# cordum-io/cordum

Measured on AMD Instinct MI355X. Metric: jobs dispatched/sec (whole node), higher is better.
Workload: dtype int64-bitset/int32 (control-plane integer path); 1 GPU; model=cordum control-plane dispatch pipeline (echo workers), global_batch=16384, seq_len=256, parallelism=shard1, rules=1024, workers_per_rank=1000, denied_jobs=14465

## Files before the change

cordum_amd/ops/hip/cordum_kernels.hip:

```cpp
#include <hip/hip_runtime.h>
#include <cstdint>

#define WAVE 64
#define BLOCK 256


template <int W, int JPT>
__global__ __launch_bounds__(BLOCK) void policy_first_match_kernel(
    const long long* __restrict__ rule_any,
    const long long* __restrict__ rule_all,
    const signed char* __restrict__ rule_secrets,
    const long long* __restrict__ rule_mcp,
    const unsigned char* __restrict__ rule_mcp_any,
    const long long* __restrict__ job_any,
    const long long* __restrict__ job_all,
    const unsigned char* __restrict__ job_secrets,
    const long long* __restrict__ job_mcp,
    const unsigned char* __restrict__ job_mcp_used,
    int* __restrict__ out_first,
    int R, int J, int rules_per_chunk)
{
    const int rule_chunk_begin = blockIdx.y * rules_per_chunk;
    const int rule_chunk_end = min(R, rule_chunk_begin + rules_per_chunk);
    constexpr int ANY_W = 7 * W;
// ... 986 lines not shown
    }
}

__global__ __launch_bounds__(BLOCK) void policy_first_match_mfma_kernel(
    const signed char* __restrict__ a_pack,
    const signed char* __restrict__ b_pack,
    const int* __restrict__ cards,
    const signed char* __restrict__ rule_secrets,
    const unsigned char* __restrict__ job_secrets,
    const int* __restrict__ tile_dims,
    int* __restrict__ out_first,
    int J, int R, int tiles_per_chunk)
{
    const int lane = threadIdx.x % WAVE;
    const int jt = blockIdx.x;
    v4i afrag[1][9];
    #pragma unroll
    for (int d = 0; d < 9; ++d)
        afrag[0][d] = *(const v4i*)&a_pack[(((size_t)jt * 9 + d) * 64 + lane) * 16];
    mfma_first_match_tiles<1>(afrag, b_pack, cards, rule_secrets, job_secrets,
                              tile_dims, out_first, J, R, tiles_per_chunk);
}

template <int TJ>
__global__ __launch_bounds__(BLOCK) void policy_first_match_mfma_bits_kernel(
    const long long* __restrict__ any_bits,
    const long long* __restrict__ all_bits,
    const signed char* __restrict__ b_pack,
    const int* __restrict__ cards,
    const signed char* __restrict__ rule_secrets,
    const unsigned char* __restrict__ job_secrets,
    const int* __restrict__ tile_dims,
    int* __restrict__ out_first,
    int J, int R, int tiles_per_chunk)
{
    const int lane = threadIdx.x % WAVE;
    const int shift = (lane >> 4) * 16;
    v4i afrag[TJ][9];
    #pragma unroll
    for (int t = 0; t < TJ; ++t) {
        const int job = (blockIdx.x * TJ + t) * 16 + (lane & 15);
        #pragma unroll
        for (int d = 0; d < 9; ++d) {
            unsigned long long w = 0;
            if (job < J)
                w = (unsigned long long)(d < 7 ? any_bits[(size_t)job * 7 + d]
                                               : all_bits[(size_t)job * 2 + (d - 7)]);
            const unsigned int slice = (unsigned int)(w >> shift) & 0xFFFFu;
            #pragma unroll
            for (int q = 0; q < 4; ++q)
                afrag[t][d][q] = (int)((((slice >> (4 * q)) & 0xFu) * 0x00204081u) & 0x01010101u);
        }
    }
    mfma_first_match_tiles<TJ>(afrag, b_pack, cards, rule_secrets, job_secrets,
                               tile_dims, out_first, J, R, tiles_per_chunk);
}


__global__ __launch_bounds__(BLOCK) void policy_gate_kernel(
    const int* __restrict__ first,
    const signed char* __restrict__ decisions,
    signed char* __restrict__ out_decision,
    int* __restrict__ denied_slots,
    int* __restrict__ denied_count,
    int* __restrict__ allowed_slots,
    int* __restrict__ allowed_count,
    int J, int R)
{
// ... 889 lines not shown
}

void tick_prologue(torch::Tensor states, torch::Tensor counts,
                   c10::optional<torch::Tensor> first,
                   torch::Tensor w_active, torch::Tensor w_maxp,
                   torch::Tensor w_cpu, torch::Tensor w_gpu, torch::Tensor out_keys)
{
    CHECK_DEV(states);
    const int B = (int)states.size(0);
    const int n = (int)counts.size(0);
    const int NW = (int)out_keys.size(0);
    TORCH_CHECK(w_active.size(0) == NW && w_maxp.size(0) == NW &&
                w_cpu.size(0) == NW && w_gpu.size(0) == NW, "worker table size mismatch");
    TORCH_CHECK(!first.has_value() || first->size(0) == B, "first must be [B]");
    const int blocks = (std::max(std::max(B, n), std::max(NW, 1)) + BLOCK - 1) / BLOCK;
    hipLaunchKernelGGL(tick_prologue_kernel, dim3(blocks), dim3(BLOCK), 0, cur_stream(),
        states.data_ptr<uint8_t>(), B, counts.data_ptr<int>(), n,
        first.has_value() ? first->data_ptr<int>() : (int*)nullptr,
        w_active.data_ptr<int>(), w_maxp.data_ptr<int>(),
        w_cpu.data_ptr<float>(), w_gpu.data_ptr<float>(),
        (unsigned long long*)out_keys.data_ptr<int64_t>(), NW);
}

void policy_first_match_mfma_bits_into(
    torch::Tensor any_bits, torch::Tensor all_bits,
    torch::Tensor b_pack, torch::Tensor cards,
    torch::Tensor rule_secrets, torch::Tensor job_secrets,
    torch::Tensor tile_dims, int64_t n_rules, torch::Tensor out, int64_t job_tiles)
{
    CHECK_DEV(any_bits); CHECK_DEV(b_pack);
    CHECK_CONTIG(any_bits); CHECK_CONTIG(all_bits);
    TORCH_CHECK(job_tiles == 1 || job_tiles == 2, "job_tiles must be 1 or 2");
    TORCH_CHECK(any_bits.dim() == 3 && any_bits.size(1) == 7 && any_bits.size(2) == 1 &&
                all_bits.dim() == 3 && all_bits.size(1) == 2 && all_bits.size(2) == 1,
                "MFMA K1 needs the 1-word vocab: any [J,7,1], all [J,2,1]");
    const int J = (int)any_bits.size(0), R = (int)n_rules;
    TORCH_CHECK(all_bits.size(0) == J && job_secrets.size(0) >= J && out.size(0) >= J,
                "job tensors must cover J");
    const int TJ = (int)job_tiles;
    const int Jt = ((J + 15) / 16 + TJ - 1) / TJ;
    const int Rt = (R + 15) / 16;
    if (J == 0 || R == 0) return;
    TORCH_CHECK(b_pack.size(0) >= Rt && tile_dims.size(0) >= Rt &&
                rule_secrets.size(0) >= Rt * 16 && cards.size(0) >= Rt * 16,
                "rule pack smaller than n_rules");
    int nchunks = std::max(1, std::min((Rt + 3) / 4, std::max(1, 2048 / std::max(Jt, 1))));
    const int tiles_per_chunk = (Rt + nchunks - 1) / nchunks;
    auto launch = [&](auto kernel) {
        hipLaunchKernelGGL(kernel, dim3(Jt, nchunks), dim3(BLOCK), 0, cur_stream(),
            (const long long*)any_bits.data_ptr<int64_t>(),
            (const long long*)all_bits.data_ptr<int64_t>(),
            (const signed char*)b_pack.data_ptr<int8_t>(),
            cards.data_ptr<int>(),
            (const signed char*)rule_secrets.data_ptr<int8_t>(),
            job_secrets.data_ptr<uint8_t>(),
            tile_dims.data_ptr<int>(),
            out.data_ptr<int>(), J, R, tiles_per_chunk);
    };
    if (TJ == 2) launch(policy_first_match_mfma_bits_kernel<2>);
    else launch(policy_first_match_mfma_bits_kernel<1>);
}

void gate_route(torch::Tensor first, torch::Tensor decisions, torch::Tensor out_decision,
                torch::Tensor denied_slots, torch::Tensor denied_count,
                torch::Tensor allowed_slots, torch::Tensor allowed_count,
                torch::Tensor states, torch::Tensor deadlines,
                torch::Tensor dlq_ring, torch::Tensor dlq_head,
                torch::Tensor pick, torch::Tensor order, torch::Tensor valid_count,
                torch::Tensor j_poolmask, torch::Tensor j_labels,
                int64_t full_mask, int64_t K,
                torch::Tensor routable_slots, torch::Tensor routable_widx,
                torch::Tensor routable_count, torch::Tensor extra_zero)
{
    CHECK_DEV(first);
    const int J = (int)first.size(0);
    TORCH_CHECK(out_decision.size(0) >= J && denied_slots.size(0) >= J &&
                allowed_slots.size(0) >= J && states.size(0) >= J &&
                deadlines.size(0) >= J && pick.size(0) >= J &&
                j_poolmask.size(0) >= J && j_labels.size(0) >= J &&
                routable_slots.size(0) >= J && routable_widx.size(0) >= J,
                "per-job tensors must cover J");
    TORCH_CHECK(K <= order.size(0), "K exceeds the order table");
    const int n_extra = (int)extra_zero.size(0);
// ... 388 lines not shown
            arow[dim_topic * W + w] = ol[o_idx * W + w];
            arow[dim_risk * W + w] = has_risk ? rl[r_idx * W + w] : 0;
            lrow[all_requires * W + w] = has_req ? ql[q_idx * W + w] : 0;
        }
    }
}

void synthetic_fresh_stamped(torch::Tensor any_bits,
                             torch::Tensor all_bits,
                             torch::Tensor tenant_lut, torch::Tensor topic_lut,
                             torch::Tensor risk_lut, torch::Tensor req_lut,
                             int64_t seed, int64_t step,
                             int64_t dim_tenant, int64_t dim_topic, int64_t dim_risk,
                             int64_t all_requires,
                             c10::optional<torch::Tensor> payload,
                             int64_t payload_words,
                             int64_t threads, int64_t isa_cap)
{
    TORCH_CHECK(!any_bits.is_cuda() && !all_bits.is_cuda(),
                "synthetic_fresh_stamped is a host encoder");
    CHECK_CONTIG(any_bits); CHECK_CONTIG(all_bits);
    CHECK_CONTIG(tenant_lut); CHECK_CONTIG(topic_lut);
    CHECK_CONTIG(risk_lut); CHECK_CONTIG(req_lut);
    cordum_enc::EncodeJob a;
    a.B = any_bits.size(0);
    a.W = any_bits.size(2);
    a.V = tenant_lut.size(0);
    TORCH_CHECK(any_bits.size(1) == 7 && all_bits.size(0) == a.B &&
                all_bits.size(1) == 2 && all_bits.size(2) == a.W, "bad batch shape");
    for (const torch::Tensor* l : {&tenant_lut, &topic_lut, &risk_lut, &req_lut})
        TORCH_CHECK(l->size(0) == a.V && l->size(1) == a.W, "bad LUT shape");
    TORCH_CHECK(dim_tenant >= 0 && dim_tenant < 7 && dim_topic >= 0 && dim_topic < 7 &&
                dim_risk >= 0 && dim_risk < 7 && all_requires >= 0 && all_requires < 2,
                "dim index out of range");
    a.any = any_bits.data_ptr<int64_t>();
    a.all = all_bits.data_ptr<int64_t>();
    a.tenant_lut = tenant_lut.data_ptr<int64_t>();
    a.topic_lut = topic_lut.data_ptr<int64_t>();
    a.risk_lut = risk_lut.data_ptr<int64_t>();
    a.req_lut = req_lut.data_ptr<int64_t>();
    a.seed = (uint64_t)seed;
    a.step = (uint64_t)step;
    a.dim_tenant = (int)dim_tenant;
    a.dim_topic = (int)dim_topic;
    a.dim_risk = (int)dim_risk;
    a.all_requires = (int)all_requires;
    a.payload = nullptr;
    a.payload_words = payload_words;
    if (payload.has_value()) {
        TORCH_CHECK(!payload->is_cuda() && payload->is_contiguous() &&
                    payload->scalar_type() == torch::kInt32 && payload_words > 0 &&
                    payload->numel() >= a.B * payload_words, "bad payload ring buffer");
        a.payload = payload->data_ptr<int32_t>();
    }
    cordum_enc::encode_batch(a, (int)threads, (int)isa_cap);
}

void pack_jobs_mfma_dev(torch::Tensor any_bits, torch::Tensor all_bits,
                        torch::Tensor a_pack)
{
    const int B = (int)any_bits.size(0);
    const int Jt = (int)a_pack.size(0);
    const int n = Jt * 9 * 64;
    const int blocks = (n + BLOCK - 1) / BLOCK;
    hipLaunchKernelGGL(pack_jobs_mfma_kernel, dim3(blocks), dim3(BLOCK), 0, cur_stream(),
        (const long long*)any_bits.data_ptr<int64_t>(),
        (const long long*)all_bits.data_ptr<int64_t>(),
        a_pack.data_ptr<int8_t>(), B, Jt);
}

// ... 27 lines not shown
    m.def("load_feedback", &load_feedback, "per-worker active-count histogram");
    m.def("run_readiness", &run_readiness, "K3 run/step readiness sweep");
    m.def("synthetic_fresh", &synthetic_fresh,
          py::call_guard<py::gil_scoped_release>(),
          "fused host synthetic-batch encoder");
    m.def("pack_jobs_mfma_dev", &pack_jobs_mfma_dev, "device job packing for the MFMA K1");
    m.def("synthetic_fresh_stamped", &synthetic_fresh_stamped,
          py::call_guard<py::gil_scoped_release>(),
          "host batch preparation in one call: synthetic dims + payload step stamp",
          py::arg("any_bits"), py::arg("all_bits"), py::arg("tenant_lut"),
          py::arg("topic_lut"), py::arg("risk_lut"), py::arg("req_lut"),
          py::arg("seed"), py::arg("step"), py::arg("dim_tenant"), py::arg("dim_topic"),
          py::arg("dim_risk"), py::arg("all_requires"), py::arg("payload"),
          py::arg("payload_words"), py::arg("threads") = 1, py::arg("isa_cap") = -1);
    m.def("encoder_isa_level", [] { return cordum_enc::max_isa_level(); },
          "widest encoder ISA this CPU runs (0 baseline, 1 AVX2, 2 AVX-512DQ)");
    m.def("tick_prologue", &tick_prologue,
          "fused tick 1/5: PENDING re-admit + counter reset + first prime + worker keys");
    m.def("policy_first_match_mfma_bits_into", &policy_first_match_mfma_bits_into,
          "fused tick 3/5: K1 MFMA with A fragments built from the staged bit words",
          py::arg("any_bits"), py::arg("all_bits"), py::arg("b_pack"), py::arg("cards"),
          py::arg("rule_secrets"), py::arg("job_secrets"), py::arg("tile_dims"),
          py::arg("n_rules"), py::arg("out"), py::arg("job_tiles") = 1);
    m.def("gate_route", &gate_route,
          "fused tick 4/5: gate + DENIED/DLQ + spread/exact pick + routable compaction");
    m.def("tick_finish", &tick_finish,
          "fused tick 5/5: echo + state chain + load feedback + counter fold");
    m.def("pack_by_dest", &pack_by_dest, "padded per-destination dispatch pack");
    m.def("pack_requeue", &pack_requeue, "redeliver last tick's requeue ring into the send segments");
    m.def("wf_sweep", &wf_sweep, "K3-WF readiness sweep + approval holds + condition/delay commits");
    m.def("wf_expand", &wf_expand, "K3-WF for_each/worker child expansion into the child arena");
    m.def("wf_apply", &wf_apply, "K3-WF child result application with failure injection");
    m.def("wf_apply_dead", &wf_apply_dead, "K3-WF dead-letter child application");
    m.def("wf_commit", &wf_commit, "K3-WF step aggregation + retry/backoff commit");
    m.def("wf_timeout_scan", &wf_timeout_scan, "K4-WF stale-step timeout scan");
    m.def("wf_readmit", &wf_readmit, "K3-WF continuous run re-admission from template");
    m.def("wf_status", &wf_status, "K3-WF run status roll-up");
    m.def("wf_grant", &wf_grant, "K3-WF host approval grants");
    m.def("materialize_rq_payload", &materialize_rq_payload, "copy requeued payload rows into the rq arena");
    m.def("gather_payload_padded", &gather_payload_padded, "payload gather into padded send arena");
    m.def("echo_padded", &echo_padded, "region-valid echo over padded recv arena");
    m.def("apply_transitions_padded", &apply_transitions_padded, "K5 over padded slot list");
    m.def("load_feedback_padded", &load_feedback_padded, "padded per-worker load histogram");
    m.def("set_transition_lut", &set_transition_lut, "upload transition legality LUT");
    m.def("apply_transitions", &apply_transitions, "K5 batched state transitions");
    m.def("deadline_scan", &deadline_scan, "K4 deadline/staleness scan");
// ... 3 lines not shown
```

cordum_amd/ops/hip/synthetic_encode.h:

```cpp
#pragma once

#include <cstddef>
#include <cstdint>
#include <thread>

namespace cordum_enc {

struct EncodeJob {
    int64_t* any;
    int64_t* all;
    const int64_t* tenant_lut;
    const int64_t* topic_lut;
    const int64_t* risk_lut;
    const int64_t* req_lut;
    int64_t B, W, V;
    uint64_t seed, step;
    int dim_tenant, dim_topic, dim_risk, all_requires;
    int32_t* payload;
    int64_t payload_words;
};

constexpr int kBlock = 64;
constexpr uint32_t kRiskCut = 1288490189u;
constexpr uint32_t kReqCut = 429496730u;

static inline uint64_t splitmix64(uint64_t x) {
    x += 0x9E3779B97F4A7C15ull;
    x = (x ^ (x >> 30)) * 0xBF58476D1CE4E5B9ull;
    x = (x ^ (x >> 27)) * 0x94D049BB133111EBull;
    return x ^ (x >> 31);
}

static inline uint64_t batch_base(uint64_t seed, uint64_t step) {
    return splitmix64(seed * 0x5851F42D4C957F2Dull ^ step);
}

__attribute__((always_inline)) static inline void encode_range_impl(
    const EncodeJob& a, int64_t i0, int64_t i1)
{
    const uint64_t base = batch_base(a.seed, a.step);
    const uint64_t v = (uint64_t)a.V;
    const int64_t W = a.W;
    const int32_t stamp = (int32_t)(uint32_t)a.step;
    uint32_t t_idx[kBlock], o_idx[kBlock], r_idx[kBlock], q_idx[kBlock];
    uint32_t c_risk[kBlock], c_req[kBlock];
    for (int64_t b0 = i0; b0 < i1; b0 += kBlock) {
        const int n = (int)((i1 - b0) < kBlock ? (i1 - b0) : kBlock);
        for (int k = 0; k < kBlock; ++k) {
            const uint64_t h0 = splitmix64(base ^ (uint64_t)(b0 + k));
            const uint64_t h1 = splitmix64(h0);
            const uint64_t h2 = splitmix64(h1);
            t_idx[k] = (uint32_t)(((h0 & 0xffffffffull) * v) >> 32);
            o_idx[k] = (uint32_t)(((h0 >> 32) * v) >> 32);
            r_idx[k] = (uint32_t)(((h1 & 0xffffffffull) * v) >> 32);
            q_idx[k] = (uint32_t)(((h1 >> 32) * v) >> 32);
            c_risk[k] = (uint32_t)h2;
            c_req[k] = (uint32_t)(h2 >> 32);
        }
        if (W == 1) {
            int64_t* arow = a.any + (size_t)b0 * 7;
            int64_t* lrow = a.all + (size_t)b0 * 2;
            for (int k = 0; k < n; ++k, arow += 7, lrow += 2) {
                arow[a.dim_tenant] = a.tenant_lut[t_idx[k]];
                arow[a.dim_topic] = a.topic_lut[o_idx[k]];
                arow[a.dim_risk] = c_risk[k] < kRiskCut ? a.risk_lut[r_idx[k]] : 0;
                lrow[a.all_requires] = c_req[k] < kReqCut ? a.req_lut[q_idx[k]] : 0;
            }
        } else {
            for (int k = 0; k < n; ++k) {
                int64_t* arow = a.any + (size_t)(b0 + k) * 7 * W;
                int64_t* lrow = a.all + (size_t)(b0 + k) * 2 * W;
                const bool has_risk = c_risk[k] < kRiskCut;
                const bool has_req = c_req[k] < kReqCut;
                const int64_t* tl = a.tenant_lut + (size_t)t_idx[k] * W;
                const int64_t* ol = a.topic_lut + (size_t)o_idx[k] * W;
                const int64_t* rl = a.risk_lut + (size_t)r_idx[k] * W;
                const int64_t* ql = a.req_lut + (size_t)q_idx[k] * W;
                for (int64_t w = 0; w < W; ++w) {
                    arow[a.dim_tenant * W + w] = tl[w];
                    arow[a.dim_topic * W + w] = ol[w];
                    arow[a.dim_risk * W + w] = has_risk ? rl[w] : 0;
                    lrow[a.all_requires * W + w] = has_req ? ql[w] : 0;
// ... 62 lines not shown
```

cordum_amd/ops/pipeline.py:

```python
from __future__ import annotations

import time
from dataclasses import dataclass
from typing import List, Optional

import torch
import torch.distributed as dist

from ..protocol.states import transition_lut
from ..safety import policy as pol
from . import get_ext
from .policy_compile import CompiledPolicy, JobBatch, JobEncoder, compile_policy, first_match_reference

UNSPECIFIED, PENDING, APPROVAL, SCHEDULED, DISPATCHED, RUNNING = 0, 1, 2, 3, 4, 5
SUCCEEDED, FAILED, CANCELLED, TIMEOUT, DENIED = 6, 7, 8, 9, 10

ALLOW_CODES = (1, 5)


@dataclass
class TickStats:
    completed: int = 0
    denied: int = 0
    unrouted: int = 0
# ... 43 lines not shown

    def __init__(self, compiled: CompiledPolicy, vocab: int = 48, seed: int = 5):
        from .policy_compile import ALL_REQUIRES, DIM_RISK, DIM_TENANT, DIM_TOPIC

        enc = JobEncoder(compiled)
        W = compiled.words
        rows = []
        for v in range(vocab):
            jb = enc.encode([
                pol.PolicyInput(tenant=f"t{v}", topic=f"job.a{v}",
                                risk_tags=[f"tag{v}"], requires=[f"req{v}"])
            ])
            rows.append(jb)
        self.W = W
        self.vocab = vocab
        self.tenant_lut = torch.stack([r.any_bits[0, DIM_TENANT] for r in rows])
        self.topic_lut = torch.stack([r.any_bits[0, DIM_TOPIC] for r in rows])
        self.risk_lut = torch.stack([r.any_bits[0, DIM_RISK] for r in rows])
        self.req_lut = torch.stack([r.all_bits[0, ALL_REQUIRES] for r in rows])
        self.gen = torch.Generator().manual_seed(seed)
        self.seed = seed
        self._dims = (DIM_TENANT, DIM_TOPIC, DIM_RISK, ALL_REQUIRES)
        self._bufs = None

    def _scratch(self, J: int):
        if self._bufs is not None and self._bufs[0].shape[0] == J:
            return self._bufs
        W = self.W
        self._bufs = (
            torch.zeros(J, dtype=torch.int64),
            torch.zeros(J, dtype=torch.int64),
            torch.zeros(J, dtype=torch.int64),
            torch.zeros(J, dtype=torch.int64),
            torch.zeros(J, dtype=torch.float32),
            torch.zeros(J, dtype=torch.float32),
            torch.zeros((J, W), dtype=torch.int64),
            torch.zeros((J, 1), dtype=torch.int64),
        )
        return self._bufs

    def fresh(self, out: JobBatch) -> None:
        DIM_TENANT, DIM_TOPIC, DIM_RISK, ALL_REQUIRES = self._dims
        J = out.n_jobs
        g = self.gen
        t_idx, o_idx, r_idx, q_idx, u_risk, u_req, row, mask = self._scratch(J)
        t_idx.random_(0, self.vocab, generator=g)
# ... 24 lines not shown
        DIM_TENANT, DIM_TOPIC, DIM_RISK, ALL_REQUIRES = self._dims
        ext.synthetic_fresh(out.any_bits, out.all_bits,
                            self.tenant_lut, self.topic_lut,
                            self.risk_lut, self.req_lut,
                            self.seed, step,
                            DIM_TENANT, DIM_TOPIC, DIM_RISK, ALL_REQUIRES)

    encode_threads = 1

    def fresh_stamped(self, out: JobBatch, step: int, ext, payload: torch.Tensor,
                      payload_words: int, threads: Optional[int] = None,
                      isa_cap: int = -1) -> None:
        DIM_TENANT, DIM_TOPIC, DIM_RISK, ALL_REQUIRES = self._dims
        ext.synthetic_fresh_stamped(out.any_bits, out.all_bits,
                                    self.tenant_lut, self.topic_lut,
                                    self.risk_lut, self.req_lut,
                                    self.seed, step,
                                    DIM_TENANT, DIM_TOPIC, DIM_RISK, ALL_REQUIRES,
                                    payload, payload_words,
                                    self.encode_threads if threads is None else threads,
                                    isa_cap)


class _RefOps:

    def __init__(self):
        self._lut = None

    def set_transition_lut(self, lut):
        self._lut = lut

    def policy_first_match(self, rule_any, rule_all, rule_secrets, rule_mcp, rule_mcp_any,
                           job_any, job_all, job_secrets, job_mcp, job_mcp_used, chunks):
        from types import SimpleNamespace

        c = SimpleNamespace(any_masks=rule_any, all_masks=rule_all, secrets=rule_secrets,
                            mcp_masks=rule_mcp, mcp_any=rule_mcp_any,
                            n_rules=int(rule_any.shape[0]))
        b = SimpleNamespace(any_bits=job_any, all_bits=job_all, secrets=job_secrets,
                            mcp_bits=job_mcp, mcp_used=job_mcp_used,
                            n_jobs=int(job_any.shape[0]))
        return first_match_reference(c, b)

    def worker_precompute(self, w_pool, w_active, w_maxp, w_cpu, w_gpu):
        from .reference import worker_precompute_ref

# ... 254 lines not shown
    nbytes = ((n64 * 8 + 2 * B + 7) // 8) * 8
    if pin:
        buf = torch.zeros(nbytes, dtype=torch.uint8).pin_memory()
    else:
        buf = torch.zeros(nbytes, dtype=torch.uint8, device=device)
    o = 0

    def take64(*shape):
        nonlocal o
        n = 1
        for s in shape:
            n *= s
        t = buf[o:o + n * 8].view(torch.int64).view(*shape)
        o += n * 8
        return t

    any_b = take64(B, 7, W)
    all_b = take64(B, 2, W)
    mcp_b = take64(B, 4, W)
    sec = buf[o:o + B]
    o += B
    used = buf[o:o + B]
    return JobBatch(any_b, all_b, sec, mcp_b, used), buf


def alloc_result_block(B: int, device=None, pin: bool = False):
    nbytes = ((4 * B + 16 + B + 7) // 8) * 8
    if pin:
        buf = torch.zeros(nbytes, dtype=torch.uint8).pin_memory()
    else:
        buf = torch.zeros(nbytes, dtype=torch.uint8, device=device)
    sums = buf[0:4 * B].view(torch.int32)
    counts = buf[4 * B:4 * B + 16].view(torch.int32)
    dec = buf[4 * B + 16:5 * B + 16].view(torch.int8)
    return sums, counts, dec, buf


class DevicePipeline:
    def __init__(
        self,
        device: torch.device,
        batch_size: int = 16384,
        n_local_workers: int = 1000,
        n_rules: int = 1024,
        payload_words: int = 64,
        world_size: int = 1,
        rank: int = 0,
        n_batches: int = 8,
        policy: Optional[pol.SafetyPolicy] = None,
        seed: int = 7,
        backend: str = "ext",
        use_mfma: Optional[bool] = None,
        mfma_pack_on_device: bool = False,
        pad_cap: Optional[int] = None,
        unfused_tick: bool = False,
        k1_job_tiles: int = 2,
    ):
        self._k1_job_tiles = k1_job_tiles
        self._pad_cap_override = pad_cap
        self._unfused_tick = unfused_tick
        self._mfma_device_pack = mfma_pack_on_device
        device = torch.device(device)
        self.ext = _RefOps() if backend == "ref" else get_ext(required=True)
        self.device = device
        self.B = batch_size
        self.NWL = n_local_workers
        self.world = world_size
        self.rank = rank
        self.payload_words = payload_words

        self.ext.set_transition_lut(torch.tensor(transition_lut(), dtype=torch.uint8).flatten())

        policy = policy or make_synthetic_policy(n_rules, seed=seed)
        for w in (1, 2, 4):
            self.compiled = compile_policy(policy, words=w)
            if self.compiled.exact:
                break
        assert self.compiled.exact, "bench policy must compile exactly"
        self.cpol = self.compiled.to(device)

# ... 98 lines not shown
            ):
                a_pack, _ = pack_jobs_mfma(jb_host)
                self.mfma_a_packs.append(a_pack.to(device))
        self._fused_capable = device.type == "cuda" and self.world == 1 and backend != "ref"
        self._tick = 0
        self.total_completed = 0
        self.total_denied = 0


    def _spread(self, pick):
        full_mask = (1 << self.world) - 1
        K = min(int(self.order_buf.shape[0]), 1024)
        self.ext.spread_pick(self.order_buf, self.valid_buf, self.j_poolmask,
                             self.j_labels, full_mask, pick, K)
        return pick

    def _refresh_order(self) -> None:
        if self._tick % 8 != 1:
            return
        self.order_buf.copy_(torch.argsort(self.w_keys).to(torch.int32))
        valid = ((self.w_keys >> 32) & 0xFFFFFFFF).ne(0xFFFFFFFE)
        self.valid_buf.copy_(valid.sum().to(torch.int32).reshape(1))

    def _fused_body(self, slot: int) -> None:
        if self._unfused_tick:
            return self._unfused_body(slot)
        B = self.B
        ext = self.ext
        jb = self.batches[slot]
        full_mask = (1 << self.world) - 1
        ext.tick_prologue(self.states, self._counts,
                          self.first_buf if self._use_mfma else None,
                          self.w_active_local, self.w_maxp,
                          self.w_cpu_local, self.w_gpu_local, self.w_keys)
        ext.least_loaded_pick_into(self.w_pool, self.w_keys, self.w_labels,
                                   self.j_poolmask, self.j_labels,
                                   self.valid_buf, full_mask, self.pick_buf)
        if self._use_mfma:
            ext.policy_first_match_mfma_bits_into(
                jb.any_bits, jb.all_bits, self.mfma_policy.b_pack,
                self.mfma_policy.cards, self.mfma_policy.secrets, jb.secrets,
                self.mfma_policy.tile_dims, self.compiled.n_rules, self.first_buf,
                self._k1_job_tiles)
            first = self.first_buf
        else:
            first = ext.policy_first_match(
                self.cpol.any_masks, self.cpol.all_masks, self.cpol.secrets,
                self.cpol.mcp_masks, self.cpol.mcp_any,
                jb.any_bits, jb.all_bits, jb.secrets, jb.mcp_bits, jb.mcp_used, 0,
            )
        K = min(int(self.order_buf.shape[0]), 1024)
        ext.gate_route(first, self.cpol.decisions, self.out_decision,
                       self.denied_slots, self.denied_count,
                       self.allowed_slots, self.allowed_count,
                       self.states, self.deadlines, self.dlq_ring, self.dlq_head,
                       self.pick_buf, self.order_buf, self.valid_buf,
                       self.j_poolmask, self.j_labels, full_mask, K,
                       self.routable_slots, self.routable_widx,
                       self.routable_count, self.w_active_local)
        ext.tick_finish(self.payloads[slot], self.routable_slots,
                        self.routable_widx, self.routable_count,
                        self.res_arena[: B * self.payload_words], self.res_sums,
                        self.payload_words,
                        self.states, self.attempts, self.deadlines,
                        [SCHEDULED, DISPATCHED, RUNNING, SUCCEEDED],
                        self.w_active_local, self.NWL, self.rank,
                        self._counts, self.acc_counts, B)

    def _unfused_body(self, slot: int) -> None:
        B = self.B
        ext = self.ext
        jb = self.batches[slot]
        if self._use_mfma:
            ext.begin_tick_first(self.states, self._counts, self.first_buf)
            if self._mfma_device_pack:
                ext.pack_jobs_mfma_dev(jb.any_bits, jb.all_bits,
                                       self.mfma_a_packs[slot])
            ext.policy_first_match_mfma_into(
                self.mfma_a_packs[slot], self.mfma_policy.b_pack, self.mfma_policy.cards,
                self.mfma_policy.secrets, jb.secrets, self.mfma_policy.tile_dims,
                self.B, self.compiled.n_rules, self.first_buf,
            )
            first = self.first_buf
# ... 76 lines not shown
        )
        self.total_completed += stats.completed
        self.total_denied += stats.denied
        return stats

    def ensure_e2e(self, seed: int = 11, payload_ring: int = 4) -> None:
        if hasattr(self, "_e2e_enc"):
            return
        assert not self._use_mfma or self._mfma_device_pack, \
            "e2e ingest needs staged descriptors: bitset K1 or device-packed MFMA"
        self._e2e_enc = SyntheticEncoder(self.compiled, seed=seed + self.rank)
        pin = self.device.type == "cuda"
        B, W = self.B, self.compiled.words

        def host(shape, dtype):
            t = torch.zeros(shape, dtype=dtype)
            return t.pin_memory() if pin else t

        self._e2e_host = JobBatch(
            host((B, 7, W), torch.int64), host((B, 2, W), torch.int64),
            host((B,), torch.uint8), host((B, 4, W), torch.int64),
            host((B,), torch.uint8),
        )
        g = torch.Generator().manual_seed(seed * 31 + self.rank)
        self._e2e_payloads = []
        for _ in range(payload_ring):
            p = torch.randint(-(1 << 31), (1 << 31) - 1,
                              (B * self.payload_words,), dtype=torch.int32, generator=g)
            self._e2e_payloads.append(p.pin_memory() if pin else p)
        self._e2e_step = 0

    def _encode_host(self, s: int, hb: JobBatch, enc: SyntheticEncoder,
                     payload: torch.Tensor) -> None:
        if hasattr(self.ext, "synthetic_fresh_stamped"):
            enc.fresh_stamped(hb, s, self.ext, payload, self.payload_words)
            return
        if hasattr(self.ext, "synthetic_fresh"):
            enc.fresh_fast(hb, s, self.ext)
        else:
            enc.fresh(hb)
        payload.view(self.B, self.payload_words)[:, 0] = s

    def tick_e2e(self) -> TickStats:
        self.ensure_e2e()
        t0 = time.perf_counter()
        step = self._e2e_step
        self._e2e_step += 1
        payload = self._e2e_payloads[step % len(self._e2e_payloads)]
        self._encode_host(step, self._e2e_host, self._e2e_enc, payload)
        nb = self.device.type == "cuda"
        jb = self.batches[0]
        jb.any_bits.copy_(self._e2e_host.any_bits, non_blocking=nb)
# ... 63 lines not shown
            if cuda:
                torch.cuda.synchronize(self.device)
            lats[s] = time.perf_counter() - t_enc[s]
        return completed, denied, lats

    def e2e_run(self, steps: int):
        self.ensure_e2e()
        if self.world > 1:
            return self._e2e_run_dist(steps)
        if self.device.type != "cuda" or not self._fused_capable:
            completed = denied = 0
            lats = []
            for _ in range(steps):
                st = self.tick_e2e()
                completed += st.completed
                denied += st.denied
                lats.append(st.wall_s)
            return completed, denied, lats

        self._ensure_graphs()
        B = self.B
        nslots = 2
        nhost = 4
        if not hasattr(self, "_e2e_hosts2"):
            Wc = self.compiled.words
            pairs = [alloc_batch_staging(B, Wc, pin=True) for _ in range(nhost)]
            self._e2e_hosts2 = [p[0] for p in pairs]
            self._e2e_host_bufs = [p[1] for p in pairs]
            self._e2e_encs = [SyntheticEncoder(self.compiled, seed=101 + 13 * i + self.rank)
                              for i in range(nhost)]
            outs = [alloc_result_block(B, pin=True) for _ in range(nslots)]
            self._e2e_out_sums = [o[0] for o in outs]
            self._e2e_out_counts = [o[1] for o in outs]
            self._e2e_out_dec = [o[2] for o in outs]
            self._e2e_out_blocks = [o[3] for o in outs]
            self._e2e_ev = [torch.cuda.Event() for _ in range(nslots)]
            self._e2e_in_ev = [torch.cuda.Event() for _ in range(nslots)]
            self._e2e_copy_stream = torch.cuda.Stream(device=self.device)
            from concurrent.futures import ThreadPoolExecutor

            self._e2e_pool = ThreadPoolExecutor(max_workers=2)

        completed = denied = 0
        lats = [0.0] * steps
        t_enc = [0.0] * steps

        def encode(s: int):
            t_enc[s] = time.perf_counter()
            self._encode_host(s, self._e2e_hosts2[s % nhost], self._e2e_encs[s % nhost],
                              self._e2e_payloads[s % len(self._e2e_payloads)])

        def harvest(s_prev: int) -> None:
            nonlocal completed, denied
            slot = s_prev % nslots
            self._e2e_ev[slot].synchronize()
            c = self._e2e_out_counts[slot]
            denied_n = int(c[0])
            routable = int(c[2])
            completed += routable
            denied += denied_n
            lats[s_prev] = time.perf_counter() - t_enc[s_prev]
            self._e2e_sums = self._e2e_out_sums[slot]
            self._e2e_decisions = self._e2e_out_dec[slot]

        futs = {}

        def submit(s: int) -> None:
            if s < steps:
                futs[s] = self._e2e_pool.submit(encode, s)

        submit(0)
        submit(1)
        for s in range(steps):
            futs.pop(s).result()
            slot = s % nslots
            with torch.cuda.stream(self._e2e_copy_stream):
                self.batch_bufs[slot].copy_(
                    self._e2e_host_bufs[s % nhost], non_blocking=True)
                self.payloads[slot].copy_(
                    self._e2e_payloads[s % len(self._e2e_payloads)],
                    non_blocking=True)
                self._e2e_in_ev[slot].record(self._e2e_copy_stream)
            torch.cuda.current_stream(self.device).wait_event(self._e2e_in_ev[slot])
            self._graphs[slot].replay()
            self._e2e_out_blocks[slot].copy_(self._res_block, non_blocking=True)
            self._e2e_ev[slot].record()
            submit(s + 2)
            if s >= 1:
                harvest(s - 1)
        harvest(steps - 1)
        return completed, denied, lats

    def tick(self) -> TickStats:
        if getattr(self, "_fused_capable", False):
            return self._tick_fused()
        if self.world > 1:
            return self._tick_padded()
        return self._tick_eager()

    def reset_stats(self) -> None:
        self.acc_counts.zero_()
        self.total_completed = 0
        self.total_denied = 0

    def tick_async(self) -> None:
        if getattr(self, "_fused_capable", False):
            self._ensure_graphs()
# ... 370 lines not shown
```

cordum_amd/ops/policy_mfma.py:

```python
from __future__ import annotations

from dataclasses import dataclass
from typing import Tuple

import torch

from .policy_compile import CompiledPolicy, JobBatch

N_DIMS = 9
VOCAB = 64


def _bits_to_onehot(words: torch.Tensor) -> torch.Tensor:
    n, d, w = words.shape
    assert w == 1, "MFMA variant supports 1-word (vocab<=64) policies"
    shifts = torch.arange(64, dtype=torch.int64)
    return ((words >> shifts.view(1, 1, 64)) & 1).to(torch.int8)


def _pack_a(onehot: torch.Tensor) -> torch.Tensor:
    J = onehot.shape[0]
    Jt = (J + 15) // 16
    padded = torch.zeros(Jt * 16, N_DIMS, VOCAB, dtype=torch.int8)
    padded[:J] = onehot
    a = padded.view(Jt, 16, N_DIMS, 4, 16)
    a = a.permute(0, 2, 3, 1, 4).reshape(Jt, N_DIMS, 64, 16)
    return a.contiguous()


def _pack_b(onehot: torch.Tensor) -> torch.Tensor:
    R = onehot.shape[0]
    Rt = (R + 15) // 16
    padded = torch.zeros(Rt * 16, N_DIMS, VOCAB, dtype=torch.int8)
    padded[:R] = onehot
    b = padded.view(Rt, 16, N_DIMS, 4, 16)
    b = b.permute(0, 2, 3, 1, 4)
    b = b.reshape(Rt, N_DIMS, 64, 16)
    return b.contiguous()


@dataclass
class MfmaPolicy:
    b_pack: torch.Tensor
    cards: torch.Tensor
    secrets: torch.Tensor
    tile_dims: torch.Tensor
    n_rules: int

    def to(self, device):
        return MfmaPolicy(self.b_pack.to(device), self.cards.to(device),
                          self.secrets.to(device), self.tile_dims.to(device),
                          self.n_rules)


def pack_policy_mfma(c: CompiledPolicy) -> MfmaPolicy:
    assert c.words == 1, "MFMA variant needs vocab <= 64"
    R = c.n_rules
    rule_bits = torch.cat([c.any_masks, c.all_masks], dim=1)
    onehot = _bits_to_onehot(rule_bits)
    b_pack = _pack_b(onehot)
    Rt = b_pack.shape[0]
    cards = torch.zeros(Rt * 16, N_DIMS, dtype=torch.int32)
    cards[:R] = onehot.sum(dim=2).to(torch.int32)
    if Rt * 16 > R:
        cards[R:, 7] = 127
    secrets = torch.full((Rt * 16,), -1, dtype=torch.int8)
    secrets[:R] = c.secrets
    used = (cards.view(Rt, 16, N_DIMS) != 0).any(dim=1)
    tile_dims = (used.to(torch.int32) << torch.arange(N_DIMS, dtype=torch.int32)).sum(
        dim=1).to(torch.int32)
    return MfmaPolicy(b_pack, cards, secrets, tile_dims, R)


def pack_jobs_mfma(jobs: JobBatch) -> Tuple[torch.Tensor, torch.Tensor]:
    job_bits = torch.cat([jobs.any_bits, jobs.all_bits], dim=1)
    onehot = _bits_to_onehot(job_bits)
    return _pack_a(onehot), jobs.secrets


def first_match_mfma(ext, mp: MfmaPolicy, a_pack: torch.Tensor,
                     job_secrets: torch.Tensor, n_jobs: int) -> torch.Tensor:
    return ext.policy_first_match_mfma(
        a_pack, mp.b_pack, mp.cards, mp.secrets, job_secrets, mp.tile_dims,
        int(n_jobs), int(mp.n_rules),
    )
```

Baseline: 110.1 million jobs/s.

## Stage jobs in compact columnar wire layout with single H2D copy per step

Adds a wire layout that holds only the policy-live dimension columns, the payload and optional secrets in one contiguous pinned buffer. The host encoder writes straight into this columnar layout, and a new MFMA K1 variant reads those columns directly. The e2e loop then does one host-to-device copy per step instead of two, through separately captured graphs. The aim is to cut PCIe bytes and host encode work for dims no rule uses, at the cost of another code path and a second set of captured graphs.

```diff
diff --git a/cordum_amd/ops/hip/cordum_kernels.hip b/cordum_amd/ops/hip/cordum_kernels.hip
--- a/cordum_amd/ops/hip/cordum_kernels.hip
+++ b/cordum_amd/ops/hip/cordum_kernels.hip
@@ -1032,7 +1032,7 @@
                               tile_dims, out_first, J, R, tiles_per_chunk);
 }
 
-template <int TJ>
+template <int TJ, bool COLS>
 __global__ __launch_bounds__(BLOCK) void policy_first_match_mfma_bits_kernel(
     const long long* __restrict__ any_bits,
     const long long* __restrict__ all_bits,
@@ -1042,7 +1042,7 @@
     const unsigned char* __restrict__ job_secrets,
     const int* __restrict__ tile_dims,
     int* __restrict__ out_first,
-    int J, int R, int tiles_per_chunk)
+    int J, int R, int tiles_per_chunk, unsigned live)
 {
     const int lane = threadIdx.x % WAVE;
     const int shift = (lane >> 4) * 16;
@@ -1053,7 +1053,11 @@
         #pragma unroll
         for (int d = 0; d < 9; ++d) {
             unsigned long long w = 0;
-            if (job < J)
+            if (COLS) {
+                if (job < J && ((live >> d) & 1u))
+                    w = (unsigned long long)any_bits[
+                        (size_t)__builtin_popcount(live & ((1u << d) - 1u)) * J + job];
+            } else if (job < J)
                 w = (unsigned long long)(d < 7 ? any_bits[(size_t)job * 7 + d]
                                                : all_bits[(size_t)job * 2 + (d - 7)]);
             const unsigned int slice = (unsigned int)(w >> shift) & 0xFFFFu;
@@ -1989,21 +1993,16 @@
         (unsigned long long*)out_keys.data_ptr<int64_t>(), NW);
 }
 
-void policy_first_match_mfma_bits_into(
-    torch::Tensor any_bits, torch::Tensor all_bits,
+static void launch_mfma_bits(
+    const long long* words, const long long* all_words, bool cols, unsigned live, int J,
     torch::Tensor b_pack, torch::Tensor cards,
     torch::Tensor rule_secrets, torch::Tensor job_secrets,
     torch::Tensor tile_dims, int64_t n_rules, torch::Tensor out, int64_t job_tiles)
 {
-    CHECK_DEV(any_bits); CHECK_DEV(b_pack);
-    CHECK_CONTIG(any_bits); CHECK_CONTIG(all_bits);
+    CHECK_DEV(b_pack);
     TORCH_CHECK(job_tiles == 1 || job_tiles == 2, "job_tiles must be 1 or 2");
-    TORCH_CHECK(any_bits.dim() == 3 && any_bits.size(1) == 7 && any_bits.size(2) == 1 &&
-                all_bits.dim() == 3 && all_bits.size(1) == 2 && all_bits.size(2) == 1,
-                "MFMA K1 needs the 1-word vocab: any [J,7,1], all [J,2,1]");
-    const int J = (int)any_bits.size(0), R = (int)n_rules;
-    TORCH_CHECK(all_bits.size(0) == J && job_secrets.size(0) >= J && out.size(0) >= J,
-                "job tensors must cover J");
+    const int R = (int)n_rules;
+    TORCH_CHECK(job_secrets.size(0) >= J && out.size(0) >= J, "job tensors must cover J");
     const int TJ = (int)job_tiles;
     const int Jt = ((J + 15) / 16 + TJ - 1) / TJ;
     const int Rt = (R + 15) / 16;
@@ -2015,17 +2014,59 @@
     const int tiles_per_chunk = (Rt + nchunks - 1) / nchunks;
     auto launch = [&](auto kernel) {
         hipLaunchKernelGGL(kernel, dim3(Jt, nchunks), dim3(BLOCK), 0, cur_stream(),
-            (const long long*)any_bits.data_ptr<int64_t>(),
-            (const long long*)all_bits.data_ptr<int64_t>(),
+            words, all_words,
             (const signed char*)b_pack.data_ptr<int8_t>(),
             cards.data_ptr<int>(),
             (const signed char*)rule_secrets.data_ptr<int8_t>(),
             job_secrets.data_ptr<uint8_t>(),
             tile_dims.data_ptr<int>(),
-            out.data_ptr<int>(), J, R, tiles_per_chunk);
+            out.data_ptr<int>(), J, R, tiles_per_chunk, live);
     };
-    if (TJ == 2) launch(policy_first_match_mfma_bits_kernel<2>);
-    else launch(policy_first_match_mfma_bits_kernel<1>);
+    if (cols) {
+        if (TJ == 2) launch(policy_first_match_mfma_bits_kernel<2, true>);
+        else launch(policy_first_match_mfma_bits_kernel<1, true>);
+    } else {
+        if (TJ == 2) launch(policy_first_match_mfma_bits_kernel<2, false>);
+        else launch(policy_first_match_mfma_bits_kernel<1, false>);
+    }
+}
+
+void policy_first_match_mfma_bits_into(
+    torch::Tensor any_bits, torch::Tensor all_bits,
+    torch::Tensor b_pack, torch::Tensor cards,
+    torch::Tensor rule_secrets, torch::Tensor job_secrets,
+    torch::Tensor tile_dims, int64_t n_rules, torch::Tensor out, int64_t job_tiles)
+{
+    CHECK_DEV(any_bits);
+    CHECK_CONTIG(any_bits); CHECK_CONTIG(all_bits);
+    TORCH_CHECK(any_bits.dim() == 3 && any_bits.size(1) == 7 && any_bits.size(2) == 1 &&
+                all_bits.dim() == 3 && all_bits.size(1) == 2 && all_bits.size(2) == 1,
+                "MFMA K1 needs the 1-word vocab: any [J,7,1], all [J,2,1]");
+    const int J = (int)any_bits.size(0);
+    TORCH_CHECK(all_bits.size(0) == J, "job tensors must cover J");
+    launch_mfma_bits((const long long*)any_bits.data_ptr<int64_t>(),
+                     (const long long*)all_bits.data_ptr<int64_t>(), false, 0u, J,
+                     b_pack, cards, rule_secrets, job_secrets, tile_dims, n_rules, out,
+                     job_tiles);
+}
+
+void policy_first_match_mfma_cols_into(
+    torch::Tensor cols, int64_t live,
+    torch::Tensor b_pack, torch::Tensor cards,
+    torch::Tensor rule_secrets, torch::Tensor job_secrets,
+    torch::Tensor tile_dims, int64_t n_rules, torch::Tensor out, int64_t job_tiles)
+{
+    CHECK_DEV(cols); CHECK_CONTIG(cols);
+    TORCH_CHECK(cols.scalar_type() == torch::kInt64 && cols.dim() == 2,
+                "cols must be int64 [n_live, J]");
+    TORCH_CHECK(live >= 0 && live < (1 << 9), "live is a 9-bit dim mask");
+    TORCH_CHECK(cols.size(0) == __builtin_popcount((unsigned)live),
+                "cols needs one row per live dim");
+    CHECK_DEV(job_secrets);
+    launch_mfma_bits((const long long*)cols.data_ptr<int64_t>(), nullptr, true,
+                     (unsigned)live, (int)cols.size(1),
+                     b_pack, cards, rule_secrets, job_secrets, tile_dims, n_rules, out,
+                     job_tiles);
 }
 
 void gate_route(torch::Tensor first, torch::Tensor decisions, torch::Tensor out_decision,
@@ -2460,7 +2501,7 @@
     CHECK_CONTIG(any_bits); CHECK_CONTIG(all_bits);
     CHECK_CONTIG(tenant_lut); CHECK_CONTIG(topic_lut);
     CHECK_CONTIG(risk_lut); CHECK_CONTIG(req_lut);
-    cordum_enc::EncodeJob a;
+    cordum_enc::EncodeJob a{};
     a.B = any_bits.size(0);
     a.W = any_bits.size(2);
     a.V = tenant_lut.size(0);
@@ -2484,6 +2525,62 @@
     a.dim_risk = (int)dim_risk;
     a.all_requires = (int)all_requires;
     a.payload = nullptr;
+    a.payload_words = payload_words;
+    if (payload.has_value()) {
+        TORCH_CHECK(!payload->is_cuda() && payload->is_contiguous() &&
+                    payload->scalar_type() == torch::kInt32 && payload_words > 0 &&
+                    payload->numel() >= a.B * payload_words, "bad payload ring buffer");
+        a.payload = payload->data_ptr<int32_t>();
+    }
+    cordum_enc::encode_batch(a, (int)threads, (int)isa_cap);
+}
+
+void synthetic_fresh_wire(torch::Tensor cols,
+                          int64_t row_tenant, int64_t row_topic,
+                          int64_t row_risk, int64_t row_req,
+                          torch::Tensor tenant_lut, torch::Tensor topic_lut,
+                          torch::Tensor risk_lut, torch::Tensor req_lut,
+                          int64_t seed, int64_t step,
+                          c10::optional<torch::Tensor> payload,
+                          int64_t payload_words,
+                          int64_t threads, int64_t isa_cap)
+{
+    TORCH_CHECK(!cols.is_cuda(), "synthetic_fresh_wire is a host encoder");
+    CHECK_CONTIG(cols);
+    CHECK_CONTIG(tenant_lut); CHECK_CONTIG(topic_lut);
+    CHECK_CONTIG(risk_lut); CHECK_CONTIG(req_lut);
+    TORCH_CHECK(cols.scalar_type() == torch::kInt64 && cols.dim() == 2,
+                "cols must be int64 [n_live, B]");
+    cordum_enc::EncodeJob a{};
+    a.B = cols.size(1);
+    a.W = 1;
+    a.V = tenant_lut.size(0);
+    for (const torch::Tensor* l : {&tenant_lut, &topic_lut, &risk_lut, &req_lut})
+        TORCH_CHECK(l->scalar_type() == torch::kInt64 && l->dim() == 2 &&
+                    l->size(0) == a.V && l->size(1) == 1, "bad LUT shape");
+    const int64_t n_live = cols.size(0);
+    int64_t* base = n_live > 0 ? cols.data_ptr<int64_t>() : nullptr;
+    auto column = [&](int64_t row) -> int64_t* {
+        TORCH_CHECK(row < n_live, "column row out of range");
+        return row < 0 ? nullptr : base + row * a.B;
+    };
+    {
+        const int64_t rows[4] = {row_tenant, row_topic, row_risk, row_req};
+        for (int i = 0; i < 4; ++i)
+            for (int j = i + 1; j < 4; ++j)
+                TORCH_CHECK(rows[i] < 0 || rows[i] != rows[j], "two dims share a column row");
+    }
+    a.columnar = true;
+    a.col_tenant = column(row_tenant);
+    a.col_topic = column(row_topic);
+    a.col_risk = column(row_risk);
+    a.col_req = column(row_req);
+    a.tenant_lut = tenant_lut.data_ptr<int64_t>();
+    a.topic_lut = topic_lut.data_ptr<int64_t>();
+    a.risk_lut = risk_lut.data_ptr<int64_t>();
+    a.req_lut = req_lut.data_ptr<int64_t>();
+    a.seed = (uint64_t)seed;
+    a.step = (uint64_t)step;
     a.payload_words = payload_words;
     if (payload.has_value()) {
         TORCH_CHECK(!payload->is_cuda() && payload->is_contiguous() &&
@@ -2557,6 +2654,19 @@
           py::arg("any_bits"), py::arg("all_bits"), py::arg("b_pack"), py::arg("cards"),
           py::arg("rule_secrets"), py::arg("job_secrets"), py::arg("tile_dims"),
           py::arg("n_rules"), py::arg("out"), py::arg("job_tiles") = 1);
+    m.def("policy_first_match_mfma_cols_into", &policy_first_match_mfma_cols_into,
+          "fused tick 3/5 on the e2e wire buffer: K1 MFMA reading the live dim columns",
+          py::arg("cols"), py::arg("live"), py::arg("b_pack"), py::arg("cards"),
+          py::arg("rule_secrets"), py::arg("job_secrets"), py::arg("tile_dims"),
+          py::arg("n_rules"), py::arg("out"), py::arg("job_tiles") = 1);
+    m.def("synthetic_fresh_wire", &synthetic_fresh_wire,
+          py::call_guard<py::gil_scoped_release>(),
+          "host batch preparation into the wire layout: live dim columns + payload stamp",
+          py::arg("cols"), py::arg("row_tenant"), py::arg("row_topic"),
+          py::arg("row_risk"), py::arg("row_req"), py::arg("tenant_lut"),
+          py::arg("topic_lut"), py::arg("risk_lut"), py::arg("req_lut"),
+          py::arg("seed"), py::arg("step"), py::arg("payload"),
+          py::arg("payload_words"), py::arg("threads") = 1, py::arg("isa_cap") = -1);
     m.def("gate_route", &gate_route,
           "fused tick 4/5: gate + DENIED/DLQ + spread/exact pick + routable compaction");
     m.def("tick_finish", &tick_finish,
diff --git a/cordum_amd/ops/hip/synthetic_encode.h b/cordum_amd/ops/hip/synthetic_encode.h
--- a/cordum_amd/ops/hip/synthetic_encode.h
+++ b/cordum_amd/ops/hip/synthetic_encode.h
@@ -18,6 +18,11 @@
     int dim_tenant, dim_topic, dim_risk, all_requires;
     int32_t* payload;
     int64_t payload_words;
+    bool columnar = false;
+    int64_t* col_tenant = nullptr;
+    int64_t* col_topic = nullptr;
+    int64_t* col_risk = nullptr;
+    int64_t* col_req = nullptr;
 };
 
 constexpr int kBlock = 64;
@@ -57,7 +62,41 @@
             c_risk[k] = (uint32_t)h2;
             c_req[k] = (uint32_t)(h2 >> 32);
         }
-        if (W == 1) {
+        if (a.columnar && a.col_tenant != nullptr && a.col_topic != nullptr &&
+            a.col_risk != nullptr && a.col_req != nullptr) {
+            int64_t* __restrict__ c0 = a.col_tenant + b0;
+            int64_t* __restrict__ c1 = a.col_topic + b0;
+            int64_t* __restrict__ c2 = a.col_risk + b0;
+            int64_t* __restrict__ c3 = a.col_req + b0;
+#if defined(__clang__)
+#pragma clang loop vectorize(disable) interleave(disable)
+#endif
+            for (int k = 0; k < n; ++k) {
+                c0[k] = a.tenant_lut[t_idx[k]];
+                c1[k] = a.topic_lut[o_idx[k]];
+                c2[k] = c_risk[k] < kRiskCut ? a.risk_lut[r_idx[k]] : 0;
+                c3[k] = c_req[k] < kReqCut ? a.req_lut[q_idx[k]] : 0;
+            }
+        } else if (a.columnar) {
+            if (a.col_tenant != nullptr) {
+                int64_t* c = a.col_tenant + b0;
+                for (int k = 0; k < n; ++k) c[k] = a.tenant_lut[t_idx[k]];
+            }
+            if (a.col_topic != nullptr) {
+                int64_t* c = a.col_topic + b0;
+                for (int k = 0; k < n; ++k) c[k] = a.topic_lut[o_idx[k]];
+            }
+            if (a.col_risk != nullptr) {
+                int64_t* c = a.col_risk + b0;
+                for (int k = 0; k < n; ++k)
+                    c[k] = c_risk[k] < kRiskCut ? a.risk_lut[r_idx[k]] : 0;
+            }
+            if (a.col_req != nullptr) {
+                int64_t* c = a.col_req + b0;
+                for (int k = 0; k < n; ++k)
+                    c[k] = c_req[k] < kReqCut ? a.req_lut[q_idx[k]] : 0;
+            }
+        } else if (W == 1) {
             int64_t* arow = a.any + (size_t)b0 * 7;
             int64_t* lrow = a.all + (size_t)b0 * 2;
             for (int k = 0; k < n; ++k, arow += 7, lrow += 2) {
diff --git a/cordum_amd/ops/pipeline.py b/cordum_amd/ops/pipeline.py
--- a/cordum_amd/ops/pipeline.py
+++ b/cordum_amd/ops/pipeline.py
@@ -89,6 +89,7 @@
         self.seed = seed
         self._dims = (DIM_TENANT, DIM_TOPIC, DIM_RISK, ALL_REQUIRES)
         self._bufs = None
+        self._wire_rows = None
 
     def _scratch(self, J: int):
         if self._bufs is not None and self._bufs[0].shape[0] == J:
@@ -159,6 +160,22 @@
                                     isa_cap)
 
 
+    def fresh_wire(self, cols: torch.Tensor, layout, step: int, ext,
+                   payload: torch.Tensor, payload_words: int,
+                   threads: Optional[int] = None, isa_cap: int = -1) -> None:
+        if self._wire_rows is None or self._wire_rows[0] != layout.live:
+            DIM_TENANT, DIM_TOPIC, DIM_RISK, ALL_REQUIRES = self._dims
+            self._wire_rows = (layout.live,
+                               layout.row(DIM_TENANT), layout.row(DIM_TOPIC),
+                               layout.row(DIM_RISK), layout.row(7 + ALL_REQUIRES))
+        ext.synthetic_fresh_wire(cols, *self._wire_rows[1:],
+                                 self.tenant_lut, self.topic_lut,
+                                 self.risk_lut, self.req_lut,
+                                 self.seed, step, payload, payload_words,
+                                 self.encode_threads if threads is None else threads,
+                                 isa_cap)
+
+
 class _RefOps:
 
     def __init__(self):
@@ -459,6 +476,24 @@
     o += B
     used = buf[o:o + B]
     return JobBatch(any_b, all_b, sec, mcp_b, used), buf
+
+
+def alloc_wire_staging(layout, B: int, payload_words: int, device=None,
+                       pin: bool = False):
+    nbytes = max(8, ((layout.offsets(B, payload_words)[2] + 7) // 8) * 8)
+    if pin:
+        buf = torch.zeros(nbytes, dtype=torch.uint8).pin_memory()
+    else:
+        buf = torch.zeros(nbytes, dtype=torch.uint8, device=device)
+    return wire_views(layout, buf, B, payload_words)
+
+
+def wire_views(layout, buf: torch.Tensor, B: int, payload_words: int):
+    o_payload, o_secrets, end = layout.offsets(B, payload_words)
+    cols = buf[0:o_payload].view(torch.int64).view(layout.n_live, B)
+    payload = buf[o_payload:o_secrets].view(torch.int32)
+    secrets = buf[o_secrets:end] if layout.has_secrets else None
+    return cols, payload, secrets, buf
 
 
 def alloc_result_block(B: int, device=None, pin: bool = False):
@@ -492,7 +527,9 @@
         pad_cap: Optional[int] = None,
         unfused_tick: bool = False,
         k1_job_tiles: int = 2,
+        wire_staging: bool = True,
     ):
+        self._wire_staging = wire_staging
         self._k1_job_tiles = k1_job_tiles
         self._pad_cap_override = pad_cap
         self._unfused_tick = unfused_tick
@@ -637,8 +674,9 @@
         valid = ((self.w_keys >> 32) & 0xFFFFFFFF).ne(0xFFFFFFFE)
         self.valid_buf.copy_(valid.sum().to(torch.int32).reshape(1))
 
-    def _fused_body(self, slot: int) -> None:
+    def _fused_body(self, slot: int, wire=None) -> None:
         if self._unfused_tick:
+            assert wire is None
             return self._unfused_body(slot)
         B = self.B
         ext = self.ext
@@ -651,7 +689,16 @@
         ext.least_loaded_pick_into(self.w_pool, self.w_keys, self.w_labels,
                                    self.j_poolmask, self.j_labels,
                                    self.valid_buf, full_mask, self.pick_buf)
-        if self._use_mfma:
+        if wire is not None:
+            w_cols, w_payload, w_secrets = wire
+            ext.policy_first_match_mfma_cols_into(
+                w_cols, self.mfma_policy.wire.live, self.mfma_policy.b_pack,
+                self.mfma_policy.cards, self.mfma_policy.secrets,
+                jb.secrets if w_secrets is None else w_secrets,
+                self.mfma_policy.tile_dims, self.compiled.n_rules, self.first_buf,
+                self._k1_job_tiles)
+            first = self.first_buf
+        elif self._use_mfma:
             ext.policy_first_match_mfma_bits_into(
                 jb.any_bits, jb.all_bits, self.mfma_policy.b_pack,
                 self.mfma_policy.cards, self.mfma_policy.secrets, jb.secrets,
@@ -673,7 +720,8 @@
                        self.j_poolmask, self.j_labels, full_mask, K,
                        self.routable_slots, self.routable_widx,
                        self.routable_count, self.w_active_local)
-        ext.tick_finish(self.payloads[slot], self.routable_slots,
+        ext.tick_finish(self.payloads[slot] if wire is None else wire[1],
+                        self.routable_slots,
                         self.routable_widx, self.routable_count,
                         self.res_arena[: B * self.payload_words], self.res_sums,
                         self.payload_words,
@@ -796,12 +844,24 @@
             host((B,), torch.uint8), host((B, 4, W), torch.int64),
             host((B,), torch.uint8),
         )
+        self._e2e_wire = (self._wire_staging and self._use_mfma and pin
+                          and self._fused_capable and not self._unfused_tick
+                          and payload_ring == 4)
+        if self._e2e_wire:
+            layout = self.mfma_policy.wire
+            self._wire_hosts = [alloc_wire_staging(layout, B, self.payload_words, pin=True)
+                                for _ in range(payload_ring)]
         g = torch.Generator().manual_seed(seed * 31 + self.rank)
         self._e2e_payloads = []
-        for _ in range(payload_ring):
+        for i in range(payload_ring):
             p = torch.randint(-(1 << 31), (1 << 31) - 1,
                               (B * self.payload_words,), dtype=torch.int32, generator=g)
-            self._e2e_payloads.append(p.pin_memory() if pin else p)
+            if self._e2e_wire:
+                self._wire_hosts[i][1].copy_(p)
+                p = self._wire_hosts[i][1]
+            elif pin:
+                p = p.pin_memory()
+            self._e2e_payloads.append(p)
         self._e2e_step = 0
 
     def _encode_host(self, s: int, hb: JobBatch, enc: SyntheticEncoder,
@@ -911,9 +971,11 @@
         B = self.B
         nslots = 2
         nhost = 4
-        if not hasattr(self, "_e2e_hosts2"):
+        wire = self._e2e_wire
+        if not hasattr(self, "_e2e_encs"):
             Wc = self.compiled.words
-            pairs = [alloc_batch_staging(B, Wc, pin=True) for _ in range(nhost)]
+            pairs = [alloc_batch_staging(B, Wc, pin=True)
+                     for _ in range(0 if wire else nhost)]
             self._e2e_hosts2 = [p[0] for p in pairs]
             self._e2e_host_bufs = [p[1] for p in pairs]
             self._e2e_encs = [SyntheticEncoder(self.compiled, seed=101 + 13 * i + self.rank)
@@ -929,6 +991,22 @@
             from concurrent.futures import ThreadPoolExecutor
 
             self._e2e_pool = ThreadPoolExecutor(max_workers=2)
+            self._e2e_stage_copies = 0
+        if wire and not hasattr(self, "_wire_devs"):
+            assert len(self._wire_hosts) == nhost
+            layout = self.mfma_policy.wire
+            self._wire_devs = [alloc_wire_staging(layout, B, self.payload_words,
+                                                  device=self.device)
+                               for _ in range(nslots)]
+            self._wire_graphs = []
+            torch.cuda.synchronize(self.device)
+            for slot in range(nslots):
+                g = torch.cuda.CUDAGraph()
+                with torch.cuda.graph(g):
+                    self._fused_body(slot, wire=self._wire_devs[slot][:3])
+                self._wire_graphs.append(g)
+            torch.cuda.synchronize(self.device)
+        graphs = self._wire_graphs if wire else self._graphs
 
         completed = denied = 0
         lats = [0.0] * steps
@@ -936,6 +1014,11 @@
 
         def encode(s: int):
             t_enc[s] = time.perf_counter()
+            if wire:
+                self._e2e_encs[s % nhost].fresh_wire(
+                    self._wire_hosts[s % nhost][0], self.mfma_policy.wire, s,
+                    self.ext, self._wire_hosts[s % nhost][1], self.payload_words)
+                return
             self._encode_host(s, self._e2e_hosts2[s % nhost], self._e2e_encs[s % nhost],
                               self._e2e_payloads[s % len(self._e2e_payloads)])
 
@@ -964,14 +1047,20 @@
             futs.pop(s).result()
             slot = s % nslots
             with torch.cuda.stream(self._e2e_copy_stream):
-                self.batch_bufs[slot].copy_(
-                    self._e2e_host_bufs[s % nhost], non_blocking=True)
-                self.payloads[slot].copy_(
-                    self._e2e_payloads[s % len(self._e2e_payloads)],
-                    non_blocking=True)
+                if wire:
+                    self._wire_devs[slot][3].copy_(
+                        self._wire_hosts[s % nhost][3], non_blocking=True)
+                    self._e2e_stage_copies += 1
+                else:
+                    self.batch_bufs[slot].copy_(
+                        self._e2e_host_bufs[s % nhost], non_blocking=True)
+                    self.payloads[slot].copy_(
+                        self._e2e_payloads[s % len(self._e2e_payloads)],
+                        non_blocking=True)
+                    self._e2e_stage_copies += 2
                 self._e2e_in_ev[slot].record(self._e2e_copy_stream)
             torch.cuda.current_stream(self.device).wait_event(self._e2e_in_ev[slot])
-            self._graphs[slot].replay()
+            graphs[slot].replay()
             self._e2e_out_blocks[slot].copy_(self._res_block, non_blocking=True)
             self._e2e_ev[slot].record()
             submit(s + 2)
diff --git a/cordum_amd/ops/policy_mfma.py b/cordum_amd/ops/policy_mfma.py
--- a/cordum_amd/ops/policy_mfma.py
+++ b/cordum_amd/ops/policy_mfma.py
@@ -1,7 +1,7 @@
 from __future__ import annotations
 
 from dataclasses import dataclass
-from typing import Tuple
+from typing import Optional, Tuple
 
 import torch
 
@@ -39,6 +39,30 @@
     return b.contiguous()
 
 
+@dataclass(frozen=True)
+class WireLayout:
+    live: int
+    has_secrets: bool
+
+    @property
+    def n_live(self) -> int:
+        return bin(self.live).count("1")
+
+    @property
+    def dims(self) -> Tuple[int, ...]:
+        return tuple(d for d in range(N_DIMS) if (self.live >> d) & 1)
+
+    def row(self, d: int) -> int:
+        if not (self.live >> d) & 1:
+            return -1
+        return bin(self.live & ((1 << d) - 1)).count("1")
+
+    def offsets(self, B: int, payload_words: int) -> Tuple[int, int, int]:
+        o_payload = self.n_live * B * 8
+        o_secrets = o_payload + B * payload_words * 4
+        return o_payload, o_secrets, o_secrets + (B if self.has_secrets else 0)
+
+
 @dataclass
 class MfmaPolicy:
     b_pack: torch.Tensor
@@ -46,11 +70,12 @@
     secrets: torch.Tensor
     tile_dims: torch.Tensor
     n_rules: int
+    wire: WireLayout
 
     def to(self, device):
         return MfmaPolicy(self.b_pack.to(device), self.cards.to(device),
                           self.secrets.to(device), self.tile_dims.to(device),
-                          self.n_rules)
+                          self.n_rules, self.wire)
 
 
 def pack_policy_mfma(c: CompiledPolicy) -> MfmaPolicy:
@@ -69,7 +94,20 @@
     used = (cards.view(Rt, 16, N_DIMS) != 0).any(dim=1)
     tile_dims = (used.to(torch.int32) << torch.arange(N_DIMS, dtype=torch.int32)).sum(
         dim=1).to(torch.int32)
-    return MfmaPolicy(b_pack, cards, secrets, tile_dims, R)
+    live_dims = (cards[:R] != 0).any(dim=0).tolist()
+    wire = WireLayout(sum(1 << d for d in range(N_DIMS) if live_dims[d]),
+                      bool((c.secrets >= 0).any()))
+    return MfmaPolicy(b_pack, cards, secrets, tile_dims, R, wire)
+
+
+def gather_wire(jobs: JobBatch, layout: WireLayout, cols: torch.Tensor,
+                secrets: Optional[torch.Tensor] = None) -> None:
+    assert jobs.any_bits.shape[2] == 1, "wire layout is the 1-word vocab"
+    dense = torch.cat([jobs.any_bits, jobs.all_bits], dim=1)[:, :, 0]
+    for r, d in enumerate(layout.dims):
+        cols[r].copy_(dense[:, d])
+    if layout.has_secrets:
+        secrets.copy_(jobs.secrets)
 
 
 def pack_jobs_mfma(jobs: JobBatch) -> Tuple[torch.Tensor, torch.Tensor]:
```

Measured after the change: 134.8 million jobs/s, median of 5. +22.5%, better.
